# ShMonem/animSnapBases

Hardware: AMD Instinct MI355X
Metric: snapshots/sec (SVD+SPLOCS) for n_verts x n_frames; basis Frobenius err vs ref (higher is better)
Workload: dtype f64

## Files before the change

### animsnapbases_amd/csrc/asb_project.hip

```cpp
#include "asb_kernels.h"

#include <algorithm>
#include <atomic>
#include <chrono>
#include <cstdlib>

typedef double d4 __attribute__((ext_vector_type(4)));

#define ASB_NBINS 2048

enum { SC_NORMX2 = 0, SC_E0MAX = 1, SC_EMAX = 2, SC_LO = 3, SC_HI = 4, SC_ABOVE = 5, SC_TAU = 6, SC_OVERFLOW = 7,
       SC_TAU_HI = 11, SC_TAU2 = 12, SC_BANDMAX = 13, SC_TAUG = 16, SC_GG = 24, SC_HH = 32,
       SC_TAU_DIV = 40, SC_DIV_SEED = 41 };
#define ASB_NG 6
__device__ __forceinline__ double guess_score(double ev, double m, double s, double g, double h) { return ev + g * m + h * s; }
__device__ __forceinline__ bool in_guess(double e, double ev, const double* __restrict__ sc) {
    const double m = e - ev, s = sqrt(fmax(m, 0.0) * fmax(ev, 0.0));
    bool in = false;
#pragma unroll
    for (int q = 0; q < ASB_NG; ++q) in = in || (guess_score(ev, m, s, sc[SC_GG + q], sc[SC_HH + q]) > sc[SC_TAUG + q]);
    return in;
}
static inline bool diverse_on(const asb_ctx* ctx) {
    return ctx->diverse && (!ctx->ev_valid || ctx->ev_cv2 > 0.5);
}
#define ASB_DIV_Q (ASB_NG + 1)
#define ASB_NQ (ASB_NG + 2)
__device__ __forceinline__ double div_key(double e, long long i, double seed_bits) {
    unsigned long long x = ((unsigned long long)i + 1ull) * 0x9E3779B97F4A7C15ull ^ (unsigned long long)__double_as_longlong(seed_bits);
    x ^= x >> 30; x *= 0xBF58476D1CE4E5B9ull; x ^= x >> 27; x *= 0x94D049BB133111EBull; x ^= x >> 31;
    const double u = ((double)(x >> 11) + 0.5) * (1.0 / 9007199254740992.0);
    return sqrt(sqrt(fmax(e, 0.0))) / -log(u);
}
__device__ __forceinline__ bool in_div(double e, long long i, const double* __restrict__ sc) {
    const double t = sc[SC_TAU_DIV];
    return t < 1.0e299 && div_key(e, i, sc[SC_DIV_SEED]) > t;
}
__global__ void k_sc_set(double* __restrict__ sc, int slot, double v) { sc[slot] = v; }

template <int T, int E2, int CPT = 1>
__global__ __launch_bounds__((T >= 256 ? T : 256)) void k_gather(
    const double* __restrict__ X, const long long* __restrict__ idx_map, long long v0, long long n_items,
    const PanelState* __restrict__ panel, const double* __restrict__ comps, long long comp_stride,
    const double* __restrict__ W, int k0, int F2, double* __restrict__ dst, double* __restrict__ energy_out,
    double* __restrict__ pmax, long long* __restrict__ pidx, double* __restrict__ psum) {
    constexpr int BLOCK = (T >= 256 ? T : 256);
    constexpr int VPB = BLOCK / T;
    constexpr int NW = T / 64;
    const int tid = threadIdx.x, g = tid / T, t = tid % T, wig = t >> 6, lane = tid & 63;
    __shared__ double red[VPB][NW];
    __shared__ double lead_e[VPB];
    __shared__ long long lead_i[VPB];
    __shared__ double lead_s[VPB];
    if (panel != nullptr && panel->n_cand < n_items) n_items = panel->n_cand;
    double bmax = -1.0, bsum = 0.0;
    long long bidx = 0x7fffffffffffffffLL;
    for (long long base = (long long)blockIdx.x * VPB * CPT; base < n_items; base += (long long)gridDim.x * VPB * CPT) {
        long long s[CPT], v[CPT];
        bool valid[CPT];
        double2 x[CPT][3][E2];
#pragma unroll
        for (int cc = 0; cc < CPT; ++cc) {
            s[cc] = base + (long long)g * CPT + cc;
            valid[cc] = s[cc] < n_items;
            v[cc] = valid[cc] ? (idx_map ? idx_map[s[cc]] - v0 : s[cc]) : 0;
            const double2* row = reinterpret_cast<const double2*>(X) + v[cc] * 3 * (long long)F2;
#pragma unroll
            for (int d = 0; d < 3; ++d)
#pragma unroll
                for (int i = 0; i < E2; ++i) {
                    const int j = t + i * T;
                    x[cc][d][i] = (valid[cc] && j < F2) ? row[(long long)d * F2 + j] : make_double2(0.0, 0.0);
                }
        }
        constexpr int U = E2 * CPT <= 4 ? 4 : (E2 * CPT <= 8 ? 2 : 1);
        for (int q0 = 0; q0 < k0; q0 += U) {
            double cf[U][CPT][3];
            double2 w[U][E2];
#pragma unroll
            for (int u = 0; u < U; ++u) {
                const int q = q0 + u < k0 ? q0 + u : k0 - 1;
                const bool on = q0 + u < k0;
#pragma unroll
                for (int cc = 0; cc < CPT; ++cc) {
                    const double* cq = comps + (long long)q * comp_stride + v[cc] * 3;
                    cf[u][cc][0] = on ? cq[0] : 0.0; cf[u][cc][1] = on ? cq[1] : 0.0; cf[u][cc][2] = on ? cq[2] : 0.0;
                }
                const double2* wq = reinterpret_cast<const double2*>(W) + (long long)q * F2;
#pragma unroll
                for (int i = 0; i < E2; ++i) {
                    const int j = t + i * T;
// ... 18 lines not shown
            double e = 0.0;
            double2* out = dst ? reinterpret_cast<double2*>(dst) + s[cc] * 3 * (long long)F2 : nullptr;
#pragma unroll
            for (int d = 0; d < 3; ++d)
#pragma unroll
                for (int i = 0; i < E2; ++i) {
                    const int j = t + i * T;
                    if (out && valid[cc] && j < F2) out[(long long)d * F2 + j] = x[cc][d][i];
                    e += x[cc][d][i].x * x[cc][d][i].x + x[cc][d][i].y * x[cc][d][i].y;
                }
            e = wave_sum(e);
            if (NW > 1) {
                __syncthreads();
                if (lane == 0) red[g][wig] = e;
                __syncthreads();
                double sum = 0.0;
#pragma unroll
                for (int q = 0; q < NW; ++q) sum += red[g][q];
                e = sum;
            }
            if (t == 0 && valid[cc]) {
                energy_out[s[cc]] = e;
                bsum += e;
                if (am_better(e, s[cc], bmax, bidx)) { bmax = e; bidx = s[cc]; }
            }
        }
    }
    if (t == 0) { lead_e[g] = bmax; lead_i[g] = bidx; lead_s[g] = bsum; }
    __syncthreads();
    if (tid == 0) {
        double be = lead_e[0], bs = lead_s[0];
        long long bi = lead_i[0];
#pragma unroll
        for (int q = 1; q < VPB; ++q) {
            bs += lead_s[q];
            if (am_better(lead_e[q], lead_i[q], be, bi)) { be = lead_e[q]; bi = lead_i[q]; }
        }
        pmax[blockIdx.x] = be; pidx[blockIdx.x] = bi; psum[blockIdx.x] = bs;
    }
}

__global__ __launch_bounds__(256) void k_range_init(const double* pmax, const long long* pidx, const double* psum,
                                                    int nblk, double* __restrict__ sc, int first) {
    __shared__ double sh_d[512];
    __shared__ long long sh_i[256];
    double be, bs;
    long long bi;
    reduce_partials(pmax, pidx, psum, nblk, sh_d, sh_i, be, bi, bs);
    if (threadIdx.x == 0) {
        sc[SC_EMAX] = be;
        sc[SC_LO] = 0.0;
        sc[SC_HI] = be;
        sc[SC_ABOVE] = 0.0;
        if (first) { sc[SC_NORMX2] = bs; sc[SC_E0MAX] = be; }
    }
}

__global__ void k_range_restore(double* __restrict__ sc, const double* __restrict__ e0) {
    sc[SC_EMAX] = e0[1];
    sc[SC_LO] = 0.0;
    sc[SC_HI] = e0[1];
    sc[SC_ABOVE] = 0.0;
    sc[SC_NORMX2] = e0[0];
    sc[SC_E0MAX] = e0[1];
}

__global__ __launch_bounds__(256) void k_hist(const double* __restrict__ E, long long n, const double* __restrict__ sc,
                                              int* __restrict__ hist, int by_exponent) {
    __shared__ int lh[ASB_NBINS];
    for (int i = threadIdx.x; i < ASB_NBINS; i += blockDim.x) lh[i] = 0;
    __syncthreads();
    const double lo = sc[SC_LO], hi = sc[SC_HI];
    const double scale = (hi > lo) ? (double)ASB_NBINS / (hi - lo) : 0.0;
    for (long long i = (long long)blockIdx.x * blockDim.x + threadIdx.x; i < n; i += (long long)gridDim.x * blockDim.x) {
        const double e = E[i];
        int b;
        if (by_exponent) {
            if (!(e >= 0.0)) continue;
            b = (int)((__double_as_longlong(e) >> 52) & 0x7FF);
        } else {
            if (e < lo || e >= hi) continue;
            b = (int)((e - lo) * scale);
            if (b > ASB_NBINS - 1) b = ASB_NBINS - 1;
        }
        atomicAdd(&lh[b], 1);
    }
    __syncthreads();
    for (int i = threadIdx.x; i < ASB_NBINS; i += blockDim.x)
        if (lh[i]) atomicAdd(&hist[i], lh[i]);
}

__device__ __forceinline__ void tau_body(int* __restrict__ hist, double* __restrict__ sc, int level, long long m_target,
                                         long long m_cap, int* lh, int* seg) {
    constexpr int PER = ASB_NBINS / 256;
    int ssum = 0;
    for (int q = 0; q < PER; ++q) {
        const int v = hist[threadIdx.x * PER + q];
        hist[threadIdx.x * PER + q] = 0;
        lh[threadIdx.x * PER + q] = v;
        ssum += v;
    }
    seg[threadIdx.x] = ssum;
    __syncthreads();
    if (threadIdx.x != 0) return;
    const double lo = sc[SC_LO], hi = sc[SC_HI];
    const double width = (hi - lo) / (double)ASB_NBINS;
    long long acc = (level == 1) ? 0 : (long long)sc[SC_ABOVE];
    int sg = 255;
    for (; sg >= 0; --sg) {
        if (acc + seg[sg] >= m_target) break;
        acc += seg[sg];
    }
    int b = -1;
    if (sg >= 0)
        for (b = sg * PER + PER - 1; b >= sg * PER; --b) {
            if (acc + lh[b] >= m_target) break;
            acc += lh[b];
        }
    if (b < 0) {
        if (level == 1) { sc[SC_LO] = 0.0; sc[SC_HI] = 0.0; sc[SC_ABOVE] = (double)acc; sc[SC_TAU] = -1.0; }
        else sc[SC_TAU] = nextafter(lo, -1.0e300);
        return;
    }
    double edge_lo, edge_hi;
    if (level == 1) {
        edge_lo = (b == 0) ? 0.0 : ldexp(1.0, b - 1023);
        edge_hi = (b >= 2046) ? 1.7976931348623157e308 : ldexp(1.0, b - 1022);
    } else {
        edge_lo = lo + b * width;
        edge_hi = (b == ASB_NBINS - 1) ? hi : lo + (b + 1) * width;
    }
    if (level == 1) {
        sc[SC_LO] = edge_lo;
        sc[SC_HI] = edge_hi;
        sc[SC_ABOVE] = (double)acc;
        sc[SC_TAU] = edge_lo;
    } else {
        double tau = edge_lo;
        if (acc + lh[b] > m_cap && acc > 0) tau = edge_hi;
        sc[SC_TAU] = nextafter(tau, -1.0e300);
    }
}

__global__ __launch_bounds__(256) void k_tau(int* __restrict__ hist, double* __restrict__ sc, int level,
                                             long long m_target, long long m_cap) {
    __shared__ int lh[ASB_NBINS];
    __shared__ int seg[256];
    tau_body(hist, sc, level, m_target, m_cap, lh, seg);
}

struct GuessTargets { double g[ASB_NQ], h[ASB_NQ]; long long m_target[ASB_NQ], m_cap[ASB_NQ]; double div_seed; };
__global__ __launch_bounds__(256) void k_hist_multi(const double* __restrict__ E, const double* __restrict__ EV, long long n,
                                                    const double* __restrict__ scm, int* __restrict__ hist, int by_exponent,
                                                    GuessTargets gt, int nq, unsigned qmask = 0xffffffffu) {
    __shared__ int lh[ASB_NBINS];
    for (int q = 0; q < nq; ++q) {
        if (!((qmask >> q) & 1u)) continue;
        for (int i = threadIdx.x; i < ASB_NBINS; i += blockDim.x) lh[i] = 0;
        __syncthreads();
        const double lo = scm[q * 8 + SC_LO], hi = scm[q * 8 + SC_HI], g = gt.g[q], h = gt.h[q];
        const double scale = (hi > lo) ? (double)ASB_NBINS / (hi - lo) : 0.0;
        for (long long i = (long long)blockIdx.x * blockDim.x + threadIdx.x; i < n; i += (long long)gridDim.x * blockDim.x) {
            double e;
            if (q == ASB_DIV_Q) e = div_key(E[i], i, gt.div_seed);
            else {
                const double ev = EV ? EV[i] : E[i], m = E[i] - ev;
                e = guess_score(ev, m, h != 0.0 ? sqrt(fmax(m, 0.0) * fmax(ev, 0.0)) : 0.0, g, h);
            }
            int b;
            if (by_exponent) {
                if (!(e >= 0.0)) continue;
                b = (int)((__double_as_longlong(e) >> 52) & 0x7FF);
            } else {
                if (e < lo || e >= hi) continue;
                b = (int)((e - lo) * scale);
                if (b > ASB_NBINS - 1) b = ASB_NBINS - 1;
            }
            atomicAdd(&lh[b], 1);
        }
        __syncthreads();
        for (int i = threadIdx.x; i < ASB_NBINS; i += blockDim.x)
            if (lh[i]) atomicAdd(&hist[q * ASB_NBINS + i], lh[i]);
        __syncthreads();
    }
}
__global__ __launch_bounds__(256) void k_tau_multi(int* __restrict__ hist, double* __restrict__ scm, double* __restrict__ sc, int level,
                                                   GuessTargets gt, unsigned qmask = 0xffffffffu) {
    __shared__ int lh[ASB_NBINS];
    __shared__ int seg[256];
    const int q = blockIdx.x;
    if (!((qmask >> q) & 1u)) {
        if (level == 2 && threadIdx.x == 0 && q < ASB_NG) { sc[SC_TAUG + q] = 1.0e300; sc[SC_GG + q] = 0.0; sc[SC_HH + q] = 0.0; }
        if (level == 2 && threadIdx.x == 0 && q == ASB_DIV_Q) sc[SC_TAU_DIV] = 1.0e300;
        return;
    }
    tau_body(hist + q * ASB_NBINS, scm + q * 8, level, gt.m_target[q], gt.m_cap[q], lh, seg);
    if (level == 2 && threadIdx.x == 0) {
        if (q == ASB_DIV_Q) {
            const double t = scm[q * 8 + SC_TAU];
            sc[SC_TAU_DIV] = t < 0.0 ? 0.0 : t;
            sc[SC_DIV_SEED] = gt.div_seed;
        } else {
            sc[q < ASB_NG ? SC_TAUG + q : SC_TAU] = scm[q * 8 + SC_TAU];
            if (q < ASB_NG) { sc[SC_GG + q] = gt.g[q]; sc[SC_HH + q] = gt.h[q]; }
        }
    }
}

#define ASB_CBLOCKS 128
__global__ __launch_bounds__(256) void k_compact_a(const double* __restrict__ E, long long n, long long v0,
                                                   const double* __restrict__ sc, int take_all, long long m_cap,
                                                   long long* __restrict__ tmp, long long* __restrict__ cnt, int hi_slot = -1,
                                                   const double* __restrict__ E2 = nullptr) {
    __shared__ long long pre[256];
    const int tid = threadIdx.x;
    const double tau = take_all ? -1.0e300 : sc[SC_TAU];
    const double tau_hi = hi_slot >= 0 ? sc[hi_slot] : 1.7976931348623157e308;
    const long long seg = (n + gridDim.x - 1) / gridDim.x;
    const long long s0 = blockIdx.x * seg, s1 = (s0 + seg < n) ? s0 + seg : n;
    const long long sub = (seg + 255) / 256;
    const long long a = s0 + tid * sub, b = (a + sub < s1) ? a + sub : s1;
    long long c = 0;
    const bool div = !take_all && hi_slot < 0;
    for (long long i = a; i < b; ++i)
        c += ((E[i] > tau && !(E[i] > tau_hi)) || (E2 && in_guess(E[i], E2[i], sc)) || (div && in_div(E[i], i, sc)));
    pre[tid] = c;
    __syncthreads();
    for (int o = 1; o < 256; o <<= 1) {
        const long long add = (tid >= o) ? pre[tid - o] : 0;
        __syncthreads();
        pre[tid] += add;
        __syncthreads();
    }
    long long pos = pre[tid] - c;
    long long* out = tmp + (long long)blockIdx.x * m_cap;
    for (long long i = a; i < b; ++i)
        if ((E[i] > tau && !(E[i] > tau_hi)) || (E2 && in_guess(E[i], E2[i], sc)) || (div && in_div(E[i], i, sc))) {
            if (pos < m_cap) out[pos] = v0 + i;
            ++pos;
        }
    if (tid == 255) cnt[blockIdx.x] = pre[255];
}

__global__ __launch_bounds__(64) void k_compact_b(const long long* __restrict__ tmp, const long long* __restrict__ cnt,
                                                  int nb, long long m_cap, long long* __restrict__ cand_idx,
                                                  PanelState* __restrict__ panel) {
    const int b = blockIdx.x;
    long long off = 0;
    for (int q = threadIdx.x; q < b; q += 64) off += cnt[q];
// ... 1214 lines not shown
    if ((rc = asb_alloc(ctx, &ctx->Wq3, (size_t)ASB_MAX_SUB * ctx->Fp * 16))) return rc;
    if ((rc = asb_alloc(ctx, &ctx->wn2t3, (size_t)16 * ASB_MAX_SUB))) return rc;
    if ((rc = asb_alloc(ctx, &ctx->tile_counter, (size_t)16))) return rc;
    const int ntile = (ncols + 15) / 16;
    WideArgs wa{};
    for (int ct = 0; ct < ntile; ++ct) {
        wa.kb[ct] = 16 * ct;
        wa.nc[ct] = ncols - 16 * ct < 16 ? ncols - 16 * ct : 16;
        hipLaunchKernelGGL(k_build_wt_fk, dim3(64), dim3(256), 0, ctx->stream, Wfk, (long long)ldw, (long long)(k0 + 16 * ct), wa.nc[ct], (int)ctx->F,
                           (int)ctx->Fp, ctx->Wt3 + (size_t)ct * ctx->Fp * 16, ctx->wn2t3 + 16 * ct, col_scale);
    }
    hipLaunchKernelGGL(k_build_wq_tiles, dim3(64, ntile), dim3(256), 0, ctx->stream, ctx->Wt3, (int)ctx->Fp, ctx->Wq3, ctx->tile_counter);
    ctx->wide_out = out_rows;
    rc = launch_wide(ctx, ntile, wa);
    ctx->wide_out = nullptr;
    return rc;
}

extern "C" int asb_test_project_columns(asb_ctx* ctx, const double* W_host, int64_t ldw, int64_t k0, int ncols, const double* col_scale_host,
                                        int path, double* out_host, int64_t out_cols) {
    if (!ctx || !ctx->X || !W_host || !out_host) return ASB_ERR_ARG;
    if (ncols < 1 || k0 < 0 || k0 + ncols > ldw || out_cols < ncols || (path != 0 && path != 1) || (path == 1 && ncols > 16 * ASB_MAX_SUB))
        ASB_FAIL(ctx, ASB_ERR_ARG, "asb_test_project_columns: ncols=%d k0=%lld ldw=%lld out_cols=%lld path=%d", ncols, (long long)k0,
                 (long long)ldw, (long long)out_cols, path);
    ASB_HIP(ctx, hipSetDevice(ctx->dev));
    const size_t rows = (size_t)3 * ctx->n_loc, nw = (size_t)ctx->F * ldw, no = (size_t)out_cols * rows;
    asb_tmp<double> W, out, sc;
    int rc = asb_test_stage(ctx, W_host, nw, 0, W);
    if (!rc) rc = asb_test_stage(ctx, out_host, no, 0, out);
    if (!rc && col_scale_host) rc = asb_test_stage(ctx, col_scale_host, (size_t)ldw, 0, sc);
    if (!rc && path == 1) rc = asb_project_columns_wide(ctx, W.get(), ldw, k0, ncols, out.get(), sc.get());
    if (path == 0)
        for (int j = 0; j < ncols && rc == ASB_OK; j += ASB_PANEL_COLS) {
            const int nc = ncols - j < ASB_PANEL_COLS ? ncols - j : ASB_PANEL_COLS;
            rc = asb_project_columns(ctx, W.get(), ldw, k0 + j, nc, out.get() + (size_t)j * rows, sc.get());
        }
    return asb_test_finish(ctx, rc, out.get(), out_host, no);
}

__global__ __launch_bounds__(256) void k_begin_reset(double* __restrict__ scal, long long n_scal, int* __restrict__ hist, int n_hist,
                                                     double* __restrict__ energy, const double* __restrict__ E0, long long n,
                                                     double* __restrict__ sc, const double* __restrict__ e0) {
    const long long i0 = (long long)blockIdx.x * 256 + threadIdx.x, st = (long long)gridDim.x * 256;
    for (long long i = i0; i < n_scal; i += st) scal[i] = 0.0;
    for (long long i = i0; i < n_hist; i += st) hist[i] = 0;
    for (long long i = i0; i < n; i += st) energy[i] = E0[i];
    if (i0 == 0) {
        sc[SC_EMAX] = e0[1];
        sc[SC_LO] = 0.0;
        sc[SC_HI] = e0[1];
        sc[SC_ABOVE] = 0.0;
        sc[SC_NORMX2] = e0[0];
        sc[SC_E0MAX] = e0[1];
    }
}

int asb_project_begin(asb_ctx* ctx, int64_t K) {
    const size_t rows = (size_t)ctx->n_loc * 3;
    int rc;
    int64_t mt = 768;
    if (const char* e = getenv("ASB_M_TARGET")) mt = atoll(e) > 16 ? atoll(e) : 16;
    ctx->m_target = ctx->N_glob < mt ? ctx->N_glob : mt;
    ctx->m_cap = ctx->N_glob < 2 * mt ? ctx->N_glob : 2 * mt;
    if ((rc = asb_alloc(ctx, &ctx->energy, (size_t)ctx->n_loc))) return rc;
    if ((rc = asb_alloc(ctx, &ctx->W, (size_t)K * ctx->Fp))) return rc;
    if ((rc = asb_alloc(ctx, &ctx->comps, (size_t)K * rows))) return rc;
    if ((rc = asb_alloc(ctx, &ctx->scal, (size_t)(K + 1) * 4))) return rc;
    if ((rc = asb_alloc(ctx, &ctx->xrec, (size_t)(2 + 3 * ctx->Fp)))) return rc;
    if ((rc = asb_alloc(ctx, &ctx->s_dev, (size_t)ctx->n_loc))) return rc;
    if ((rc = asb_alloc(ctx, &ctx->Wt, (size_t)ctx->Fp * ASB_PANEL_COLS))) return rc;
    if ((rc = asb_alloc(ctx, &ctx->wn2t, (size_t)ASB_PANEL_COLS))) return rc;
    if ((rc = asb_alloc(ctx, &ctx->candR, (size_t)ctx->m_cap * 3 * ctx->Fp))) return rc;
    if ((rc = asb_alloc(ctx, &ctx->cand_e, (size_t)ctx->m_cap))) return rc;
    if ((rc = asb_alloc(ctx, &ctx->cand_idx, (size_t)ctx->m_cap))) return rc;
    if ((rc = asb_alloc(ctx, &ctx->cpmax, (size_t)ctx->nblk_cap))) return rc;
    if ((rc = asb_alloc(ctx, &ctx->cpidx, (size_t)ctx->nblk_cap))) return rc;
    if ((rc = asb_alloc(ctx, &ctx->cpsum, (size_t)ctx->nblk_cap))) return rc;
    if ((rc = asb_alloc(ctx, &ctx->colpart, (size_t)ctx->nblk_cap * 16))) return rc;
    if ((rc = asb_alloc(ctx, &ctx->hist, (size_t)ASB_NBINS))) return rc;
    if ((rc = asb_alloc(ctx, &ctx->pstate, (size_t)1))) return rc;
    if ((rc = asb_alloc(ctx, &ctx->gram, (size_t)K * ASB_PANEL_COLS))) return rc;
    if ((rc = asb_alloc(ctx, &ctx->gram_s, (size_t)K * ASB_PANEL_COLS))) return rc;
    if ((rc = asb_alloc(ctx, &ctx->ctmp, (size_t)ASB_CBLOCKS * ctx->m_cap))) return rc;
    if ((rc = asb_alloc(ctx, &ctx->ccnt, (size_t)ASB_CBLOCKS))) return rc;
    StreamCfg c;
    if (!pick_cfg(ctx->Fp, c)) ASB_FAIL(ctx, ASB_ERR_LIMIT, "F too large");
    hipLaunchKernelGGL(k_sc_set, dim3(1), dim3(1), 0, ctx->stream, ctx->scalar_dev, (int)SC_TAU_DIV, 1.0e300);
    ctx->diverse_next = ctx->read_diverse = false;
    ctx->n_diverse_reads = 0;
    ctx->sub_cur = 0;
    for (int q = 0; q < 8; ++q) ctx->sub_budget[q] = ASB_PANEL_COLS;
    if (ctx->e0_valid && ctx->E0 && ctx->e0_reuse) {
        const long long nmax = ctx->n_loc > (K + 1) * 4 ? ctx->n_loc : (K + 1) * 4;
        hipLaunchKernelGGL(k_begin_reset, dim3((unsigned)((nmax + 255) / 256 < 2048 ? (nmax + 255) / 256 : 2048)), dim3(256), 0, ctx->stream,
                           ctx->scal, (long long)(K + 1) * 4, ctx->hist, (int)ASB_NBINS, ctx->energy, ctx->E0, (long long)ctx->n_loc,
                           ctx->scalar_dev, ctx->e0_sc);
        ASB_CHECK_LAUNCH(ctx);
        ctx->nblk = 0;
        ctx->n_energy_pass = 0;
        return ASB_OK;
    }
    ASB_HIP(ctx, hipMemsetAsync(ctx->hist, 0, ASB_NBINS * sizeof(int), ctx->stream));
    ASB_HIP(ctx, hipMemsetAsync(ctx->scal, 0, (size_t)(K + 1) * 4 * sizeof(double), ctx->stream));
    const int grid = stream_grid(ctx, c, ctx->n_loc);
    StreamArgs a{ctx->X, nullptr, nullptr, nullptr, nullptr, ctx->energy, ctx->pmax, ctx->pidx, ctx->psum,
                 (long long)ctx->n_loc, nullptr};
    launch_stream(ctx, c, false, grid, a);
    ASB_CHECK_LAUNCH(ctx);
    ctx->nblk = grid;
    hipLaunchKernelGGL(k_range_init, dim3(1), dim3(256), 0, ctx->stream, ctx->pmax, ctx->pidx, ctx->psum, ctx->nblk,
                       ctx->scalar_dev, 1);
    ASB_CHECK_LAUNCH(ctx);
    ctx->n_energy_pass = 1;
    ctx->mean_frac = 0.0;
    ctx->ev_valid = false;
    if ((rc = asb_alloc(ctx, &ctx->E0, (size_t)ctx->n_loc))) return rc;
    if ((rc = asb_alloc(ctx, &ctx->e0_sc, (size_t)4))) return rc;
    ASB_HIP(ctx, hipMemcpyAsync(ctx->E0, ctx->energy, (size_t)ctx->n_loc * sizeof(double), hipMemcpyDeviceToDevice, ctx->stream));
    ASB_HIP(ctx, hipMemcpyAsync(ctx->e0_sc, ctx->scalar_dev + SC_NORMX2, 2 * sizeof(double), hipMemcpyDeviceToDevice, ctx->stream));
    ctx->e0_valid = true;
    return ASB_OK;
}

template <int T, int E2>
__global__ __launch_bounds__((T >= 256 ? T : 256)) void k_cand_dots(
    const double* __restrict__ R0, const double* __restrict__ wk, const double* __restrict__ scal_k, int t_panel,
    long long m_cap, double* __restrict__ cand_c, double* __restrict__ energy, double* __restrict__ pmax,
    long long* __restrict__ pidx, double* __restrict__ psum, int F2, const PanelState* __restrict__ panel) {
    if (panel->done) return;
    constexpr int BLOCK = (T >= 256 ? T : 256);
    constexpr int VPB = BLOCK / T;
    constexpr int NW = T / 64;
    const int tid = threadIdx.x, g = tid / T, t = tid % T, wig = t >> 6, lane = tid & 63;
    __shared__ double red[VPB][NW][3];
    __shared__ double lead_e[VPB];
    __shared__ long long lead_i[VPB];
    const long long n = panel->n_cand;
    double2 w[E2];
#pragma unroll
    for (int i = 0; i < E2; ++i) {
// ... 146 lines not shown
                       ctx->scal + k * 4, t_panel, (long long)ctx->m_cap, ctx->cand_c, ctx->cand_e, ctx->cpmax, ctx->cpidx,
                       ctx->cpsum, (int)(ctx->Fp / 2), ctx->pstate);
}
template <int E2>
static void launch_cand_dots_e(asb_ctx* ctx, int T, int grid, long long k, int t_panel) {
    switch (T) {
        case 64: launch_cand_dots_te<64, E2>(ctx, grid, k, t_panel); break;
        case 128: launch_cand_dots_te<128, E2>(ctx, grid, k, t_panel); break;
        case 256: launch_cand_dots_te<256, E2>(ctx, grid, k, t_panel); break;
        case 512: launch_cand_dots_te<512, E2>(ctx, grid, k, t_panel); break;
        default: launch_cand_dots_te<1024, E2>(ctx, grid, k, t_panel); break;
    }
}
static void launch_cand_dots(asb_ctx* ctx, const StreamCfg& c, int grid, long long k, int t_panel) {
    switch (c.E2) {
        case 4: launch_cand_dots_e<4>(ctx, c.T, grid, k, t_panel); break;
        case 8: launch_cand_dots_e<8>(ctx, c.T, grid, k, t_panel); break;
        default: launch_cand_dots_e<16>(ctx, c.T, grid, k, t_panel); break;
    }
}

#define ASB_MARGIN_REL 1.0e-11

static int hist_grid(const asb_ctx* ctx) {
    const long long n = ctx->n_loc;
    return (int)((n + 255) / 256 < 512 ? (n + 255) / 256 : 512);
}

int asb_sketch_subset_tau(asb_ctx* ctx, const double* E, long long n, long long m_target, long long m_cap) {
    int rc;
    if ((rc = asb_alloc(ctx, &ctx->hist, (size_t)ASB_NBINS))) return rc;
    if ((rc = asb_alloc(ctx, &ctx->scalar_dev, (size_t)48))) return rc;
    ASB_HIP(ctx, hipMemsetAsync(ctx->hist, 0, ASB_NBINS * sizeof(int), ctx->stream));
    long long want = (n + 255) / 256;
    const int grid = (int)(want < 4LL * ctx->n_cu ? want : 4LL * ctx->n_cu);
    for (int level = 1; level <= 2; ++level) {
        hipLaunchKernelGGL(k_hist, dim3(grid), dim3(256), 0, ctx->stream, E, n, ctx->scalar_dev, ctx->hist, level == 1 ? 1 : 0);
        hipLaunchKernelGGL(k_tau, dim3(1), dim3(256), 0, ctx->stream, ctx->hist, ctx->scalar_dev, level, m_target, m_cap);
    }
    ASB_CHECK_LAUNCH(ctx);
    return ASB_OK;
}

extern "C" int asb_panel_hist(asb_ctx* ctx, int level, int* hist_dev) {
    if (!ctx || !ctx->energy || ctx->mode != ASB_DEFLATE_PROJECT) return ASB_ERR_ARG;
    int* h = hist_dev ? hist_dev : ctx->hist;
    if (hist_dev) ASB_HIP(ctx, hipMemsetAsync(h, 0, ASB_NBINS * sizeof(int), ctx->stream));
    hipLaunchKernelGGL(k_hist, dim3(hist_grid(ctx)), dim3(256), 0, ctx->stream, ctx->energy, (long long)ctx->n_loc,
                       ctx->scalar_dev, h, level == 1 ? 1 : 0);
    ASB_CHECK_LAUNCH(ctx);
    return ASB_OK;
}

extern "C" int asb_panel_tau(asb_ctx* ctx, int level, const int* hist_dev) {
    if (!ctx || !ctx->energy || ctx->mode != ASB_DEFLATE_PROJECT) return ASB_ERR_ARG;
    hipLaunchKernelGGL(k_tau, dim3(1), dim3(256), 0, ctx->stream, hist_dev ? const_cast<int*>(hist_dev) : ctx->hist, ctx->scalar_dev, level,
                       (long long)(ctx->m_target_eff ? ctx->m_target_eff : ctx->m_target), (long long)ctx->m_cap);
    ASB_CHECK_LAUNCH(ctx);
    return ASB_OK;
}

__global__ __launch_bounds__(256) void k_export_above(const double* __restrict__ energy, long long n, const double* __restrict__ sc,
                                                      long long cap, double* __restrict__ out, unsigned* __restrict__ counter) {
    const double tau = sc[SC_TAU];
    for (long long v = (long long)blockIdx.x * 256 + threadIdx.x; v < n; v += (long long)gridDim.x * 256) {
        const double e = energy[v];
        if (e > tau) {
            const unsigned slot = atomicAdd(counter, 1u);
            if (slot < cap) out[slot] = e;
        }
    }
    if (blockIdx.x == 0 && threadIdx.x == 0) out[cap] = tau;
}
__global__ __launch_bounds__(256) void k_fill(double* __restrict__ out, long long n, double v, unsigned* __restrict__ counter) {
    for (long long i = (long long)blockIdx.x * 256 + threadIdx.x; i < n; i += (long long)gridDim.x * 256) out[i] = v;
    if (blockIdx.x == 0 && threadIdx.x == 0) *counter = 0u;
}

extern "C" int asb_panel_top_energies(asb_ctx* ctx, double* out_dev, int64_t cap) {
    if (!ctx || !ctx->energy || ctx->mode != ASB_DEFLATE_PROJECT || !out_dev || cap < 1) return ASB_ERR_ARG;
    int rc;
    if ((rc = asb_alloc(ctx, &ctx->tile_counter, (size_t)16))) return rc;
    unsigned* counter = ctx->tile_counter + 15;
    hipLaunchKernelGGL(k_fill, dim3(8), dim3(256), 0, ctx->stream, out_dev, (long long)cap + 1, -1.0, counter);
    hipLaunchKernelGGL(k_export_above, dim3(hist_grid(ctx)), dim3(256), 0, ctx->stream, ctx->energy, (long long)ctx->n_loc,
                       ctx->scalar_dev, (long long)cap, out_dev, counter);
    ASB_CHECK_LAUNCH(ctx);
    return ASB_OK;
}

extern "C" int asb_panel_set_tau(asb_ctx* ctx, const double* tau_dev) {
    if (!ctx || !ctx->energy || ctx->mode != ASB_DEFLATE_PROJECT || !tau_dev) return ASB_ERR_ARG;
    ASB_HIP(ctx, hipMemcpyAsync(ctx->scalar_dev + SC_TAU, tau_dev, sizeof(double), hipMemcpyDeviceToDevice, ctx->stream));
    return ASB_OK;
}

extern "C" int asb_panel_select(asb_ctx* ctx, int64_t k, int64_t forced_gidx, int global_all, double* rows_out,
                                long long* idx_out, int64_t* n_local, int* overflow) {
    if (!ctx || !ctx->energy || ctx->mode != ASB_DEFLATE_PROJECT) return ASB_ERR_ARG;
    if (!pick_cfg(ctx->Fp, ctx->cfg)) ASB_FAIL(ctx, ASB_ERR_LIMIT, "F too large");
    const StreamCfg c = ctx->cfg;
    const long long n = ctx->n_loc;
    double* rows = rows_out ? rows_out : ctx->candR;
    long long* idx = idx_out ? idx_out : ctx->cand_idx;
    if (forced_gidx >= 0) {
        hipLaunchKernelGGL(k_force_single, dim3(1), dim3(1), 0, ctx->stream, (long long)forced_gidx, (long long)ctx->v0, n,
                           idx, ctx->pstate);
    } else {
        hipLaunchKernelGGL(k_compact_a, dim3(ASB_CBLOCKS), dim3(256), 0, ctx->stream, ctx->energy, n, (long long)ctx->v0,
                           ctx->scalar_dev, global_all, (long long)ctx->m_cap, ctx->ctmp, ctx->ccnt, -1, ctx->sel_e2);
        hipLaunchKernelGGL(k_compact_b, dim3(ASB_CBLOCKS), dim3(64), 0, ctx->stream, ctx->ctmp, ctx->ccnt, ASB_CBLOCKS,
                           (long long)ctx->m_cap, idx, ctx->pstate);
    }
// ... 183 lines not shown
    panel->spec_ok = ASB_PANEL_COLS;
    for (int sp = 0; sp < ASB_MAX_SUB; ++sp) {
        sub[sp] = *panel;
        sub[sp].spec_max = sp < ma.nsub ? ma.spec_max[sp] : 0;
    }
}

template <int NJ>
__global__ __launch_bounds__(256, (NJ > 16 ? 1 : 2)) void k_panel_multi(const double* __restrict__ R0, int F, int Fp,
                                                        double* __restrict__ W, double* __restrict__ scal, MultiArgs ma,
                                                        const PanelState* panel, PanelState* sub,
                                                        const long long* __restrict__ cand_idx, unsigned* __restrict__ bar,
                                                        unsigned long long* rec, unsigned long long* wbuf, unsigned long long* swbuf,
                                                        double* rows_out, int test_stall, int spec_rank) {
    constexpr int NQ = NJ / 4;
    __shared__ __attribute__((aligned(16))) double w_sh[NJ * 64 + 8];
    __shared__ double wv_e[4];
    __shared__ long long wv_i[4];
    __shared__ double sh_e[4];
    __shared__ int sh_i[4];
    __shared__ int sh_c[4];
    const int tid = threadIdx.x, lane = tid & 63, wv = tid >> 6;
    const int G = gridDim.x;
    const long long n_cand = panel->n_cand;
    if (n_cand > 4LL * G) {
        if (blockIdx.x == 0 && tid == 0) bar[2] = 1u;
        return;
    }
    const int Gact = n_cand > 0 ? (int)((n_cand + 3) / 4) : 1;
    if ((int)blockIdx.x >= Gact) return;
    const int WROW = Fp + 8;
    const double thr = panel->theta + panel->margin, e_floor = panel->margin;
    const bool overflow = panel->pad != 0;
    const long long s = (long long)blockIdx.x * 4 + wv;
    const bool have = s < n_cand && cand_idx[s] >= 0;
    double x[3][NJ];
    {
        const double* row = R0 + s * 3 * (long long)Fp;
#pragma unroll
        for (int d = 0; d < 3; ++d)
#pragma unroll
            for (int j = 0; j < NJ; ++j) {
                const int f = lane + 64 * j;
                x[d][j] = (have && f < Fp) ? row[(long long)d * Fp + f] : 0.0;
            }
    }
    if (spec_rank > 0) {
#pragma unroll
        for (int r3 = 0; r3 < 3; ++r3) {
            unsigned long long* sown = swbuf + ((size_t)r3 * G + blockIdx.x) * WROW;
            for (int f = tid; f < WROW; f += 256) coop_store_u64(sown + f, ASB_SENT_D);
        }
    }
    double g[6] = {0, 0, 0, 0, 0, 0};
#pragma unroll
    for (int j = 0; j < NJ; ++j) {
        const double a = x[0][j], b = x[1][j], c = x[2][j];
        g[0] += a * a; g[1] += a * b; g[2] += a * c; g[3] += b * b; g[4] += b * c; g[5] += c * c;
    }
    wave_sum_dpp<6>(g);
    unsigned long long* tlog = reinterpret_cast<unsigned long long*>(bar + 4);
    const long long spin_max = test_stall ? (1LL << 10) : (1LL << 20);
    int gstep = 0;
    bool aborted = false, ended = false;
    bool spec_now = false, spec_prev = false;
    int sp = 0;
    for (; sp < ma.nsub && !ended; ++sp) {
        const long long k0 = ma.kb[sp];
        const int steps = ma.steps[sp], spec_max = overflow ? 0 : ma.spec_max[sp];
        PanelState* st = sub + sp;
        int proven = -1, nrun = 0;
        for (int t = 0; t < steps; ++t, ++gstep) {
            const int ring = gstep % 3, ring_prev = (gstep + 2) % 3;
            if (blockIdx.x == 0 && tid == 0) tlog[gstep * 6 + 0] = wall_clock64();
            const double e = (g[0] + g[3]) + g[5];
            if (lane == 0) { wv_e[wv] = have ? e : -1.0; wv_i[wv] = have ? s : 0x7fffffffffffffffLL; }
            __builtin_amdgcn_s_waitcnt(0);
            __syncthreads();
            int ow = 0;
#pragma unroll
            for (int q = 1; q < 4; ++q)
                if (am_better(wv_e[q], wv_i[q], wv_e[ow], wv_i[ow])) ow = q;
            unsigned long long* myrec = rec + ((size_t)ring * G + blockIdx.x) * 2;
            if (tid == 0 && !(test_stall && (int)blockIdx.x == Gact - 1)) {
                const unsigned long long slot32 = wv_i[ow] > 0x7ffffffeLL ? 0x7fffffffull : (unsigned long long)wv_i[ow];
                coop_store(reinterpret_cast<double*>(myrec), wv_e[ow]);
                coop_store_u64(myrec + 1, slot32 | (spec_now && wv_e[ow] > 0.0 ? (1ull << 32) : 0ull));
            }
            if (blockIdx.x == 0 && tid == 0) tlog[gstep * 6 + 1] = wall_clock64();
            double lam = 0.0, u0 = 0.0, u1 = 0.0, u2 = 0.0;
            double be = -2.0;
            int bi = 0x7fffffff, dead = 0, better = 0;
            if (wv == ow) {
                if (wv_e[ow] > 0.0) {
                    eig3_top_fast(g[0], g[1], g[2], g[3], g[4], g[5], lam, u0, u1, u2);
                    double wn1[1] = {0.0};
#pragma unroll
                    for (int j = 0; j < NJ; ++j) {
                        const double wvv = u0 * x[0][j] + u1 * x[1][j] + u2 * x[2][j];
                        w_sh[lane + 64 * j] = wvv;
                        wn1[0] += wvv * wvv;
                    }
                    wave_sum_dpp<1>(wn1);
                    if (lane == 0) { w_sh[NJ * 64] = wn1[0]; w_sh[NJ * 64 + 1] = lam; }
                    if (spec_now) {
                        double* sw = reinterpret_cast<double*>(swbuf) + ((size_t)ring * G + blockIdx.x) * WROW;
#pragma unroll
                        for (int q = 0; q < NJ / 2; ++q) {
                            const int f2 = 2 * lane + 128 * q;
                            if (f2 < Fp) {
                                typedef double d2v __attribute__((ext_vector_type(2)));
                                const d2v v = *reinterpret_cast<const d2v*>(&w_sh[f2]);
                                asm volatile("global_store_dwordx4 %0, %1, off sc1" :: "v"(sw + f2), "v"(v) : "memory");
                            }
                        }
                        if (lane == 0) {
                            typedef double d2v __attribute__((ext_vector_type(2)));
                            const d2v hd2 = {wn1[0], lam};
                            asm volatile("global_store_dwordx4 %0, %1, off sc1" :: "v"(sw + Fp), "v"(hd2) : "memory");
                        }
                    }
                }
            } else {
                const unsigned long long* recs = rec + (size_t)ring * G * 2;
                const int p = (wv - (wv > ow ? 1 : 0)) * 64 + lane;
                for (int b = p; b < Gact; b += 192) {
                    unsigned long long eb, ib;
                    long long spins = 0;
                    for (;;) {
                        eb = coop_load_u64(recs + 2 * b);
                        ib = coop_load_u64(recs + 2 * b + 1);
                        if (eb != ASB_SENT_D && ib != (unsigned long long)ASB_SENT_I) break;
                        if ((++spins & 63) == 0 &&
                            (spins > spin_max || __hip_atomic_load(bar + 1, __ATOMIC_RELAXED, __HIP_MEMORY_SCOPE_AGENT))) { dead = 1; break; }
                    }
                    if (dead) break;
                    const double ebd = __longlong_as_double((long long)eb);
                    const int sl = (int)(ib & 0x7fffffffull);
                    const int ibs = sl == 0x7fffffff ? 0x7fffffff : 2 * sl + ((ib >> 32) & 1ull ? 0 : 1);
                    if (ebd > be || (ebd == be && ibs < bi)) { be = ebd; bi = ibs; }
                    if (ebd > wv_e[ow] || (ebd == wv_e[ow] && (long long)sl < wv_i[ow])) ++better;
                }
                const double em = wave_max_dpp(be);
                bi = wave_min_dpp(be == em ? bi : 0x7fffffff);
                be = em;
                better = wave_isum_dpp(better);
            }
            if (lane == 0) { sh_e[wv] = be; sh_i[wv] = bi; sh_c[wv] = better; }
// ... 49 lines not shown
                }
                if (tid < 2) coop_store(reinterpret_cast<double*>(wb) + Fp + tid, w_sh[NJ * 64 + tid]);
            } else {
                unsigned long long tmp[NQ], hd = 0ull;
                long long spins = 0;
                for (;;) {
                    bool all = true;
#pragma unroll
                    for (int q = 0; q < NQ; ++q) {
                        const int f = tid + 256 * q;
                        tmp[q] = (f < Fp) ? coop_load_u64(wb + f) : 0ull;
                        all = all && tmp[q] != ASB_SENT_D;
                    }
                    if (tid < 2) { hd = coop_load_u64(wb + Fp + tid); all = all && hd != ASB_SENT_D; }
                    if (all) break;
                    if ((++spins & 63) == 0 &&
                        (spins > spin_max || __hip_atomic_load(bar + 1, __ATOMIC_RELAXED, __HIP_MEMORY_SCOPE_AGENT))) { dead = 1; break; }
                }
#pragma unroll
                for (int q = 0; q < NQ; ++q) w_sh[tid + 256 * q] = __longlong_as_double((long long)tmp[q]);
                if (tid < 2) w_sh[NJ * 64 + tid] = __longlong_as_double((long long)hd);
            }
            if (__syncthreads_or(dead)) { aborted = true; break; }
            if (blockIdx.x == 0 && tid == 0) tlog[gstep * 6 + 3] = wall_clock64();
            const double wn2 = w_sh[NJ * 64];
            if (bb == (int)blockIdx.x) {
                const long long k = k0 + t;
                for (int f = tid; f < Fp; f += 256) W[k * (long long)Fp + f] = w_sh[f];
                if (tid == 0) {
                    scal[k * 4 + 0] = sqrt(fmax(w_sh[NJ * 64 + 1], 0.0));
                    scal[k * 4 + 1] = wn2;
                    scal[k * 4 + 2] = __longlong_as_double(cand_idx[bi]);
                    st->e_win[t] = be;
                }
            }
            if (blockIdx.x == 0 && tid == 0) st->committed = t + 1;
            if (have) {
                double acc[3] = {0.0, 0.0, 0.0};
                constexpr int JB = NJ < 8 ? NJ : 8;
#pragma unroll
                for (int jb = 0; jb < NJ; jb += JB) {
                    double wj[JB];
#pragma unroll
                    for (int u = 0; u < JB; ++u) wj[u] = w_sh[lane + 64 * (jb + u)];
#pragma unroll
                    for (int u = 0; u < JB; ++u) {
                        acc[0] += x[0][jb + u] * wj[u]; acc[1] += x[1][jb + u] * wj[u]; acc[2] += x[2][jb + u] * wj[u];
                    }
                    __builtin_amdgcn_sched_barrier(0);
                }
                wave_sum_dpp<3>(acc);
#pragma unroll
                for (int d = 0; d < 3; ++d) acc[d] /= wn2;
#pragma unroll
                for (int q = 0; q < 6; ++q) g[q] = 0.0;
#pragma unroll
                for (int jb = 0; jb < NJ; jb += JB) {
                    double wj[JB];
#pragma unroll
                    for (int u = 0; u < JB; ++u) wj[u] = w_sh[lane + 64 * (jb + u)];
#pragma unroll
                    for (int u = 0; u < JB; ++u) {
                        const int j = jb + u;
                        const double a = x[0][j] - acc[0] * wj[u], b = x[1][j] - acc[1] * wj[u], c = x[2][j] - acc[2] * wj[u];
                        x[0][j] = a; x[1][j] = b; x[2][j] = c;
                        g[0] += a * a; g[1] += a * b; g[2] += a * c; g[3] += b * b; g[4] += b * c; g[5] += c * c;
                    }
                    __builtin_amdgcn_sched_barrier(0);
                }
                wave_sum_dpp<6>(g);
            }
            if (blockIdx.x == 0 && tid == 0) tlog[gstep * 6 + 4] = wall_clock64();
        }
        if (aborted) break;
        if (blockIdx.x == 0 && tid == 0) st->proven = proven < 0 ? nrun : proven;
        if (nrun < ASB_PANEL_COLS) ended = true;
    }
    if (aborted) {
        if (tid == 0) __hip_atomic_store(bar + 1, 1u, __ATOMIC_RELAXED, __HIP_MEMORY_SCOPE_AGENT);
        return;
    }
    if (blockIdx.x == 0 && tid == 0)
        for (int q = sp; q < ma.nsub; ++q) { sub[q].proven = 0; sub[q].done = 1; }
    if (rows_out != nullptr && have) {
        double* row = rows_out + s * 3 * (long long)Fp;
#pragma unroll
        for (int d = 0; d < 3; ++d)
#pragma unroll
            for (int j = 0; j < NJ; ++j) {
                const int f = lane + 64 * j;
                if (f < Fp) row[(long long)d * Fp + f] = x[d][j];
            }
    }
}

static int coop_buffers(asb_ctx* ctx, int* cgrid_all, size_t* n_words) {
    int rc;
    *cgrid_all = (int)((ctx->m_cap + 3) / 4);
    *n_words = (size_t)3 * *cgrid_all * 2 + (size_t)3 * (ctx->Fp + 8) + (size_t)3 * *cgrid_all * (ctx->Fp + 8);
    if ((rc = asb_alloc(ctx, &ctx->coop_bar, (size_t)4 + 2 * 64 * 6))) return rc;
    return asb_alloc(ctx, &ctx->coop_rec, *n_words);
}
constexpr int SPEC_W_RANK = 24;

template <int NJ>
static int launch_panel_multi(asb_ctx* ctx, int grid, const MultiArgs& ma, bool* launched, PanelState* sub, bool writeback) {
    int per_cu = 0;
    ASB_HIP(ctx, hipOccupancyMaxActiveBlocksPerMultiprocessor(&per_cu, (const void*)k_panel_multi<NJ>, 256, 0));
    if (per_cu < 1) { *launched = false; return ASB_OK; }
    if ((long long)per_cu * ctx->n_cu < grid) grid = per_cu * ctx->n_cu;
    unsigned long long* words = (unsigned long long*)ctx->coop_rec;
    hipLaunchKernelGGL(k_panel_multi<NJ>, dim3(grid), dim3(256), 0, ctx->stream, ctx->candR, (int)ctx->F, (int)ctx->Fp, ctx->W, ctx->scal,
                       ma, ctx->pstate, sub, ctx->cand_idx, ctx->coop_bar, words, words + (size_t)3 * grid * 2,
                       words + (size_t)3 * grid * 2 + (size_t)3 * (ctx->Fp + 8), writeback ? ctx->candR : (double*)nullptr,
                       ctx->coop_test_stall, SPEC_W_RANK);
    ASB_CHECK_LAUNCH(ctx);
    *launched = true;
    ctx->n_coop_launches++;
    return ASB_OK;
}

static int launch_panel_multi_any(asb_ctx* ctx, int grid, const MultiArgs& ma, bool* launched, PanelState* sub, bool writeback) {
    if (ctx->Fp <= 256) return launch_panel_multi<4>(ctx, grid, ma, launched, sub, writeback);
// ... 1064 lines not shown
                           with_score ? ctx->sk_score : (const double*)nullptr, (long long)ctx->n_loc, ctx->scm, ctx->hist6,
                           level == 1 ? 1 : 0, gt, ASB_NQ, qmask);
        hipLaunchKernelGGL(k_tau_multi, dim3(ASB_NQ), dim3(256), 0, ctx->stream, ctx->hist6, ctx->scm, ctx->scalar_dev, level, gt, qmask);
    }
    ASB_CHECK_LAUNCH(ctx);
    return ASB_OK;
}
extern "C" int asb_panel_guess_stats(asb_ctx* ctx, double* mean_energy_local, double* normx2_local, int* possible) {
    if (!ctx || !mean_energy_local || !normx2_local || !possible) return ASB_ERR_ARG;
    *possible = guess_possible(ctx) ? 1 : 0;
    *mean_energy_local = *possible ? ctx->mean_energy : 0.0;
    *normx2_local = *possible ? ctx->prep_normx2 : 0.0;
    return ASB_OK;
}
extern "C" int asb_panel_guess_begin(asb_ctx* ctx, int world) {
    if (!ctx || !ctx->energy || ctx->mode != ASB_DEFLATE_PROJECT || world < 1) return ASB_ERR_ARG;
    if (!guess_possible(ctx)) ASB_FAIL(ctx, ASB_ERR_ARG, "asb_panel_guess_begin: no energies without the constant direction");
    int rc;
    if ((rc = guess_thresholds(ctx, world, false))) return rc;
    ctx->sel_e2 = ctx->EV;
    ctx->m_target_eff = ctx->m_target / 12;
    ctx->n_guess_panels++;
    return ASB_OK;
}
extern "C" int asb_panel_guess_end(asb_ctx* ctx) {
    if (!ctx) return ASB_ERR_ARG;
    ctx->sel_e2 = nullptr;
    ctx->m_target_eff = 0;
    return ASB_OK;
}

static int panel_candidates(asb_ctx* ctx, long long k, int stalled) {
    int rc;
    const bool guess = k == 0 && stalled == 0 && ctx->mean_frac > 0.25 && guess_possible(ctx);
    const bool by_score = ctx->sketch_valid && stalled == 0 && k > 0;
    ctx->sketch_valid = false;
    ctx->read_by_score = by_score;
    const bool div_plain = diverse_on(ctx) && ctx->diverse_next && stalled == 0 && k > 0 && ctx->n_loc > 4 * ctx->m_cap;
    ctx->diverse_next = false;
    ctx->read_diverse = false;
    if (by_score) {
        if ((rc = score_thresholds(ctx, true, diverse_on(ctx) ? ctx->m_target / 8 : 0))) return rc;
        ctx->sel_e2 = ctx->sk_score;
        ctx->n_sketch_reads++;
    } else if (guess) {
        if ((rc = guess_thresholds(ctx, 1, true))) return rc;
        ctx->sel_e2 = ctx->EV;
        ctx->n_guess_panels++;
    } else if (div_plain) {
        if ((rc = score_thresholds(ctx, false, ctx->m_target / 2))) return rc;
        ctx->read_diverse = true;
        ctx->n_diverse_reads++;
    } else {
        hipLaunchKernelGGL(k_sc_set, dim3(1), dim3(1), 0, ctx->stream, ctx->scalar_dev, (int)SC_TAU_DIV, 1.0e300);
        for (int level = 1; level <= 2; ++level) {
            if ((rc = asb_panel_hist(ctx, level, nullptr))) return rc;
            if ((rc = asb_panel_tau(ctx, level, nullptr))) return rc;
        }
    }
    return asb_panel_select(ctx, k, -1, 0, nullptr, nullptr, nullptr, nullptr);
}

__global__ void k_scal_to_direct(double* __restrict__ scal, long long k, const double* __restrict__ sc) {
    double r2 = sc[SC_NORMX2];
    for (long long j = 0; j < k; ++j) {
        r2 -= scal[j * 4 + 3];
        scal[j * 4 + 3] = r2;
    }
}
extern "C" int asb_project_switch_residual(asb_ctx* ctx, int64_t k) {
    if (!ctx || !ctx->energy || !ctx->comps || !ctx->W) return ASB_ERR_ARG;
    if (ctx->mode != ASB_DEFLATE_PROJECT) ASB_FAIL(ctx, ASB_ERR_ARG, "asb_project_switch_residual: not in projection mode");
    if (k < 0 || k > ctx->K) ASB_FAIL(ctx, ASB_ERR_ARG, "asb_project_switch_residual: k = %lld out of range", (long long)k);
    int rc;
    if ((rc = asb_alloc(ctx, &ctx->R, (size_t)ctx->n_loc * 3 * ctx->Fp))) return rc;
    if (!pick_cfg(ctx->Fp, ctx->cfg)) ASB_FAIL(ctx, ASB_ERR_LIMIT, "F too large");
    const int ggrid = stream_grid(ctx, ctx->cfg, ctx->n_loc);
    launch_gather(ctx, ctx->cfg, ggrid, nullptr, (long long)ctx->n_loc, nullptr, (int)k, ctx->R, ctx->energy, ctx->pmax, ctx->pidx,
                  ctx->psum);
    ASB_CHECK_LAUNCH(ctx);
    ctx->nblk = ggrid;
    ctx->n_refresh++;
    hipLaunchKernelGGL(k_scal_to_direct, dim3(1), dim3(1), 0, ctx->stream, ctx->scal, (long long)k, ctx->scalar_dev);
    ASB_CHECK_LAUNCH(ctx);
    ctx->mode = ASB_DEFLATE_RESIDUAL;
    ctx->local = 0;
    ctx->forced_row = -1;
    ctx->sel_e2 = nullptr;
    ctx->k_done = k;
    ctx->k_switch = k;
    if (asb_debug_panels())
        fprintf(stderr, "[asb] k=%lld: %lld reads of X so far -- the run continues in the residual loop\n", (long long)k,
                (long long)(ctx->n_panels + ctx->n_refresh));
    return ASB_OK;
}
extern "C" int asb_deflate_switch_stats(asb_ctx* ctx, int64_t* k_switch) {
    if (!ctx || !k_switch) return ASB_ERR_ARG;
    *k_switch = ctx->k_switch;
    return ASB_OK;
}
static bool stall_rule(asb_ctx* ctx, long long k) {
    if (!ctx->stall_fallback) return false;
    const long long reads = ctx->n_panels + ctx->n_refresh;
    if (reads - ctx->fb_mark_reads < 8) return false;
    const bool slow = (k - ctx->fb_mark_k) * 4 < (reads - ctx->fb_mark_reads) * 3;
    ctx->fb_mark_reads = reads;
    ctx->fb_mark_k = k;
    return slow;
}
extern "C" int asb_deflate_pick(asb_ctx* ctx, int64_t k, const double* recs_dev, int64_t n_rec);
// ... 159 lines not shown
```

Before: 447,300.

## Parallelize tau histogram scan, drop sc_set launches, defer Gram off-diagonals

Replaces the single-thread serial scan in tau_body with a wave-shuffle prefix sum across 256 threads, so the threshold bin is found in parallel without a shared-memory histogram copy. Removes the separate k_sc_set kernel launches by folding the SC_TAU_DIV reset into range init, restore and k_tau. In the streaming panel kernel, only the diagonal Gram terms are kept per step, and the off-diagonal terms are recomputed only in the owning wave when an eigen solve is needed. The aim is to cut launch count, serial latency and per-step reduction work, at the cost of an extra pass over x in the owner wave.

Result: faster. 461,200 (median of 6 runs) (+3.1%).

```diff
diff --git a/animsnapbases_amd/csrc/asb_project.hip b/animsnapbases_amd/csrc/asb_project.hip
--- a/animsnapbases_amd/csrc/asb_project.hip
+++ b/animsnapbases_amd/csrc/asb_project.hip
@@ -36,7 +36,6 @@
     const double t = sc[SC_TAU_DIV];
     return t < 1.0e299 && div_key(e, i, sc[SC_DIV_SEED]) > t;
 }
-__global__ void k_sc_set(double* __restrict__ sc, int slot, double v) { sc[slot] = v; }
 
 template <int T, int E2, int CPT = 1>
 __global__ __launch_bounds__((T >= 256 ? T : 256)) void k_gather(
@@ -161,7 +160,7 @@
         sc[SC_LO] = 0.0;
         sc[SC_HI] = be;
         sc[SC_ABOVE] = 0.0;
-        if (first) { sc[SC_NORMX2] = bs; sc[SC_E0MAX] = be; }
+        if (first) { sc[SC_NORMX2] = bs; sc[SC_E0MAX] = be; sc[SC_TAU_DIV] = 1.0e300; }
     }
 }
 
@@ -200,32 +199,51 @@
 }
 
 __device__ __forceinline__ void tau_body(int* __restrict__ hist, double* __restrict__ sc, int level, long long m_target,
-                                         long long m_cap, int* lh, int* seg) {
+                                         long long m_cap) {
     constexpr int PER = ASB_NBINS / 256;
-    int ssum = 0;
+    __shared__ long long wtot[4];
+    __shared__ long long res_acc;
+    __shared__ int res_b, res_cnt;
+    const int tid = threadIdx.x, lane = tid & 63, wv = tid >> 6;
+    int v[PER];
+    long long ssum = 0;
+#pragma unroll
     for (int q = 0; q < PER; ++q) {
-        const int v = hist[threadIdx.x * PER + q];
-        hist[threadIdx.x * PER + q] = 0;
-        lh[threadIdx.x * PER + q] = v;
-        ssum += v;
-    }
-    seg[threadIdx.x] = ssum;
+        v[q] = hist[tid * PER + q];
+        hist[tid * PER + q] = 0;
+        ssum += v[q];
+    }
+    long long incl = ssum;
+#pragma unroll
+    for (int o = 1; o < 64; o <<= 1) {
+        const long long dn = __shfl_down(incl, o, 64);
+        if (lane + o < 64) incl += dn;
+    }
+    if (lane == 0) wtot[wv] = incl;
     __syncthreads();
-    if (threadIdx.x != 0) return;
+    for (int w = wv + 1; w < 4; ++w) incl += wtot[w];
     const double lo = sc[SC_LO], hi = sc[SC_HI];
     const double width = (hi - lo) / (double)ASB_NBINS;
-    long long acc = (level == 1) ? 0 : (long long)sc[SC_ABOVE];
-    int sg = 255;
-    for (; sg >= 0; --sg) {
-        if (acc + seg[sg] >= m_target) break;
-        acc += seg[sg];
-    }
-    int b = -1;
-    if (sg >= 0)
-        for (b = sg * PER + PER - 1; b >= sg * PER; --b) {
-            if (acc + lh[b] >= m_target) break;
-            acc += lh[b];
-        }
+    const long long above = (level == 1) ? 0 : (long long)sc[SC_ABOVE];
+    incl += above;
+    const long long excl = incl - ssum;
+    if (incl >= m_target && (tid == 255 || excl < m_target)) {
+        long long acc = excl;
+        int qb = 0, cnt = v[0];
+        bool found = false;
+#pragma unroll
+        for (int q = PER - 1; q > 0; --q)
+            if (!found) {
+                if (acc + v[q] >= m_target) { found = true; qb = q; cnt = v[q]; }
+                else acc += v[q];
+            }
+        res_b = tid * PER + qb; res_acc = acc; res_cnt = cnt;
+    } else if (tid == 0 && incl < m_target) { res_b = -1; res_acc = incl; res_cnt = 0; }
+    __syncthreads();
+    if (tid != 0) return;
+    const int b = res_b;
+    const long long acc = res_acc;
+    const int cnt_b = res_cnt;
     if (b < 0) {
         if (level == 1) { sc[SC_LO] = 0.0; sc[SC_HI] = 0.0; sc[SC_ABOVE] = (double)acc; sc[SC_TAU] = -1.0; }
         else sc[SC_TAU] = nextafter(lo, -1.0e300);
@@ -246,16 +264,15 @@
         sc[SC_TAU] = edge_lo;
     } else {
         double tau = edge_lo;
-        if (acc + lh[b] > m_cap && acc > 0) tau = edge_hi;
+        if (acc + cnt_b > m_cap && acc > 0) tau = edge_hi;
         sc[SC_TAU] = nextafter(tau, -1.0e300);
     }
 }
 
 __global__ __launch_bounds__(256) void k_tau(int* __restrict__ hist, double* __restrict__ sc, int level,
-                                             long long m_target, long long m_cap) {
-    __shared__ int lh[ASB_NBINS];
-    __shared__ int seg[256];
-    tau_body(hist, sc, level, m_target, m_cap, lh, seg);
+                                             long long m_target, long long m_cap, int div_off = 0) {
+    tau_body(hist, sc, level, m_target, m_cap);
+    if (div_off && level == 2 && threadIdx.x == 0) sc[SC_TAU_DIV] = 1.0e300;
 }
 
 struct GuessTargets { double g[ASB_NQ], h[ASB_NQ]; long long m_target[ASB_NQ], m_cap[ASB_NQ]; double div_seed; };
@@ -295,15 +312,13 @@
 }
 __global__ __launch_bounds__(256) void k_tau_multi(int* __restrict__ hist, double* __restrict__ scm, double* __restrict__ sc, int level,
                                                    GuessTargets gt, unsigned qmask = 0xffffffffu) {
-    __shared__ int lh[ASB_NBINS];
-    __shared__ int seg[256];
     const int q = blockIdx.x;
     if (!((qmask >> q) & 1u)) {
         if (level == 2 && threadIdx.x == 0 && q < ASB_NG) { sc[SC_TAUG + q] = 1.0e300; sc[SC_GG + q] = 0.0; sc[SC_HH + q] = 0.0; }
         if (level == 2 && threadIdx.x == 0 && q == ASB_DIV_Q) sc[SC_TAU_DIV] = 1.0e300;
         return;
     }
-    tau_body(hist + q * ASB_NBINS, scm + q * 8, level, gt.m_target[q], gt.m_cap[q], lh, seg);
+    tau_body(hist + q * ASB_NBINS, scm + q * 8, level, gt.m_target[q], gt.m_cap[q]);
     if (level == 2 && threadIdx.x == 0) {
         if (q == ASB_DIV_Q) {
             const double t = scm[q * 8 + SC_TAU];
@@ -1624,6 +1639,7 @@
         sc[SC_ABOVE] = 0.0;
         sc[SC_NORMX2] = e0[0];
         sc[SC_E0MAX] = e0[1];
+        sc[SC_TAU_DIV] = 1.0e300;
     }
 }
 
@@ -1657,7 +1673,6 @@
     if ((rc = asb_alloc(ctx, &ctx->ccnt, (size_t)ASB_CBLOCKS))) return rc;
     StreamCfg c;
     if (!pick_cfg(ctx->Fp, c)) ASB_FAIL(ctx, ASB_ERR_LIMIT, "F too large");
-    hipLaunchKernelGGL(k_sc_set, dim3(1), dim3(1), 0, ctx->stream, ctx->scalar_dev, (int)SC_TAU_DIV, 1.0e300);
     ctx->diverse_next = ctx->read_diverse = false;
     ctx->n_diverse_reads = 0;
     ctx->sub_cur = 0;
@@ -1910,13 +1925,14 @@
     return ASB_OK;
 }
 
-extern "C" int asb_panel_tau(asb_ctx* ctx, int level, const int* hist_dev) {
+static int panel_tau(asb_ctx* ctx, int level, const int* hist_dev, int div_off) {
     if (!ctx || !ctx->energy || ctx->mode != ASB_DEFLATE_PROJECT) return ASB_ERR_ARG;
     hipLaunchKernelGGL(k_tau, dim3(1), dim3(256), 0, ctx->stream, hist_dev ? const_cast<int*>(hist_dev) : ctx->hist, ctx->scalar_dev, level,
-                       (long long)(ctx->m_target_eff ? ctx->m_target_eff : ctx->m_target), (long long)ctx->m_cap);
+                       (long long)(ctx->m_target_eff ? ctx->m_target_eff : ctx->m_target), (long long)ctx->m_cap, div_off);
     ASB_CHECK_LAUNCH(ctx);
     return ASB_OK;
 }
+extern "C" int asb_panel_tau(asb_ctx* ctx, int level, const int* hist_dev) { return panel_tau(ctx, level, hist_dev, 0); }
 
 __global__ __launch_bounds__(256) void k_export_above(const double* __restrict__ energy, long long n, const double* __restrict__ sc,
                                                       long long cap, double* __restrict__ out, unsigned* __restrict__ counter) {
@@ -2206,13 +2222,13 @@
             for (int f = tid; f < WROW; f += 256) coop_store_u64(sown + f, ASB_SENT_D);
         }
     }
-    double g[6] = {0, 0, 0, 0, 0, 0};
+    double gd[3] = {0, 0, 0};
 #pragma unroll
     for (int j = 0; j < NJ; ++j) {
         const double a = x[0][j], b = x[1][j], c = x[2][j];
-        g[0] += a * a; g[1] += a * b; g[2] += a * c; g[3] += b * b; g[4] += b * c; g[5] += c * c;
-    }
-    wave_sum_dpp<6>(g);
+        gd[0] += a * a; gd[1] += b * b; gd[2] += c * c;
+    }
+    wave_sum_dpp<3>(gd);
     unsigned long long* tlog = reinterpret_cast<unsigned long long*>(bar + 4);
     const long long spin_max = test_stall ? (1LL << 10) : (1LL << 20);
     int gstep = 0;
@@ -2227,7 +2243,7 @@
         for (int t = 0; t < steps; ++t, ++gstep) {
             const int ring = gstep % 3, ring_prev = (gstep + 2) % 3;
             if (blockIdx.x == 0 && tid == 0) tlog[gstep * 6 + 0] = wall_clock64();
-            const double e = (g[0] + g[3]) + g[5];
+            const double e = (gd[0] + gd[1]) + gd[2];
             if (lane == 0) { wv_e[wv] = have ? e : -1.0; wv_i[wv] = have ? s : 0x7fffffffffffffffLL; }
             __builtin_amdgcn_s_waitcnt(0);
             __syncthreads();
@@ -2247,7 +2263,14 @@
             int bi = 0x7fffffff, dead = 0, better = 0;
             if (wv == ow) {
                 if (wv_e[ow] > 0.0) {
-                    eig3_top_fast(g[0], g[1], g[2], g[3], g[4], g[5], lam, u0, u1, u2);
+                    double go[3] = {0, 0, 0};
+#pragma unroll
+                    for (int j = 0; j < NJ; ++j) {
+                        const double a = x[0][j], b = x[1][j], c = x[2][j];
+                        go[0] += a * b; go[1] += a * c; go[2] += b * c;
+                    }
+                    wave_sum_dpp<3>(go);
+                    eig3_top_fast(gd[0], go[0], go[1], gd[1], go[2], gd[2], lam, u0, u1, u2);
                     double wn1[1] = {0.0};
 #pragma unroll
                     for (int j = 0; j < NJ; ++j) {
@@ -2403,8 +2426,7 @@
                 wave_sum_dpp<3>(acc);
 #pragma unroll
                 for (int d = 0; d < 3; ++d) acc[d] /= wn2;
-#pragma unroll
-                for (int q = 0; q < 6; ++q) g[q] = 0.0;
+                gd[0] = gd[1] = gd[2] = 0.0;
 #pragma unroll
                 for (int jb = 0; jb < NJ; jb += JB) {
                     double wj[JB];
@@ -2415,11 +2437,11 @@
                         const int j = jb + u;
                         const double a = x[0][j] - acc[0] * wj[u], b = x[1][j] - acc[1] * wj[u], c = x[2][j] - acc[2] * wj[u];
                         x[0][j] = a; x[1][j] = b; x[2][j] = c;
-                        g[0] += a * a; g[1] += a * b; g[2] += a * c; g[3] += b * b; g[4] += b * c; g[5] += c * c;
+                        gd[0] += a * a; gd[1] += b * b; gd[2] += c * c;
                     }
                     __builtin_amdgcn_sched_barrier(0);
                 }
-                wave_sum_dpp<6>(g);
+                wave_sum_dpp<3>(gd);
             }
             if (blockIdx.x == 0 && tid == 0) tlog[gstep * 6 + 4] = wall_clock64();
         }
@@ -3590,10 +3612,9 @@
         ctx->read_diverse = true;
         ctx->n_diverse_reads++;
     } else {
-        hipLaunchKernelGGL(k_sc_set, dim3(1), dim3(1), 0, ctx->stream, ctx->scalar_dev, (int)SC_TAU_DIV, 1.0e300);
         for (int level = 1; level <= 2; ++level) {
             if ((rc = asb_panel_hist(ctx, level, nullptr))) return rc;
-            if ((rc = asb_panel_tau(ctx, level, nullptr))) return rc;
+            if ((rc = panel_tau(ctx, level, nullptr, 1))) return rc;
         }
     }
     return asb_panel_select(ctx, k, -1, 0, nullptr, nullptr, nullptr, nullptr);
```
